# GalDude33/Fetal-MRI-Segmentation

Measured on NVIDIA B200. Metric: U-Net train voxels/sec, higher is better.
Workload: dtype bf16

## Files before the change

fetal-mri-segmentation_b200/csrc/bandwidth.cu:

```cuda
#include "common.cuh"

#include <algorithm>

namespace {

constexpr int kThreads = 256;

__device__ __forceinline__ uint4 ldg16(const void* p) { return __ldg(reinterpret_cast<const uint4*>(p)); }
__device__ __forceinline__ void stg16(void* p, uint4 v) { *reinterpret_cast<uint4*>(p) = v; }

__device__ __forceinline__ void unpack8(uint4 v, float f[8]) {
  const __nv_bfloat162* h = reinterpret_cast<const __nv_bfloat162*>(&v);
#pragma unroll
  for (int i = 0; i < 4; ++i) {
    float2 t = __bfloat1622float2(h[i]);
    f[2 * i] = t.x;
    f[2 * i + 1] = t.y;
  }
}
__device__ __forceinline__ uint4 pack8(const float f[8]) {
  uint4 v;
  __nv_bfloat162* h = reinterpret_cast<__nv_bfloat162*>(&v);
#pragma unroll
  for (int i = 0; i < 4; ++i) h[i] = __floats2bfloat162_rn(f[2 * i], f[2 * i + 1]);
  return v;
}

__global__ void cast_f32_bf16_kernel(const float* __restrict__ in, bf16* __restrict__ out, int64_t n) {
  int64_t i = ((int64_t)blockIdx.x * blockDim.x + threadIdx.x) * 8;
  if (i + 8 <= n) {
    float4 a = __ldg(reinterpret_cast<const float4*>(in + i));
    float4 b = __ldg(reinterpret_cast<const float4*>(in + i + 4));
    float f[8] = {a.x, a.y, a.z, a.w, b.x, b.y, b.z, b.w};
    stg16(out + i, pack8(f));
  } else {
    for (; i < n; ++i) out[i] = __float2bfloat16(in[i]);
  }
}
__global__ void cast_bf16_f32_kernel(const bf16* __restrict__ in, float* __restrict__ out, int64_t n) {
  int64_t i = ((int64_t)blockIdx.x * blockDim.x + threadIdx.x) * 8;
  if (i + 8 <= n) {
    float f[8];
    unpack8(ldg16(in + i), f);
    *reinterpret_cast<float4*>(out + i) = make_float4(f[0], f[1], f[2], f[3]);
    *reinterpret_cast<float4*>(out + i + 4) = make_float4(f[4], f[5], f[6], f[7]);
  } else {
    for (; i < n; ++i) out[i] = __bfloat162float(in[i]);
  }
}

__global__ void pad_cast_kernel(const float* __restrict__ in, bf16* __restrict__ out, int64_t vox, int Cin, int Cpad) {
  const int64_t total = vox * Cpad;
  for (int64_t g = (int64_t)blockIdx.x * blockDim.x + threadIdx.x; g < total; g += (int64_t)gridDim.x * blockDim.x) {
    const int c = (int)(g % Cpad);
    const int64_t v = g / Cpad;
    out[g] = __float2bfloat16(c < Cin ? __ldg(in + v * Cin + c) : 0.f);
  }
}

template <int pz>
__global__ void maxpool3d_fwd_kernel(const bf16* __restrict__ x, bf16* __restrict__ y, int N, int X,
                                     int Y, int Z, int C) {
  FM_PDL_SYNC();
  const int c8n = C >> 3;
  const int Xo = X >> 1, Yo = Y >> 1, Zo = Z / pz;
  const int64_t total = (int64_t)N * Xo * Yo * Zo * c8n;
  int64_t g = (int64_t)blockIdx.x * blockDim.x + threadIdx.x;
  if (g >= total) return;
  const int c8 = (int)(g % c8n);
  int64_t v = g / c8n;
  const int zo = (int)(v % Zo);
  v /= Zo;
  const int yo = (int)(v % Yo);
  v /= Yo;
  const int xo = (int)(v % Xo);
  const int n = (int)(v / Xo);
  __nv_bfloat162 m[4];
  bool first = true;
#pragma unroll
  for (int dx = 0; dx < 2; ++dx)
#pragma unroll
    for (int dy = 0; dy < 2; ++dy)
#pragma unroll
      for (int dz = 0; dz < 2; ++dz) {
        if (dz >= pz) continue;
        const int64_t vi = (((int64_t)n * X + 2 * xo + dx) * Y + 2 * yo + dy) * Z + pz * zo + dz;
        uint4 t = ldg16(x + vi * C + c8 * 8);
        const __nv_bfloat162* h = reinterpret_cast<const __nv_bfloat162*>(&t);
        if (first) {
#pragma unroll
          for (int i = 0; i < 4; ++i) m[i] = h[i];
          first = false;
        } else {
#pragma unroll
          for (int i = 0; i < 4; ++i) m[i] = __hmax2(m[i], h[i]);
        }
      }
  uint4 o;
  __nv_bfloat162* oh = reinterpret_cast<__nv_bfloat162*>(&o);
#pragma unroll
  for (int i = 0; i < 4; ++i) oh[i] = m[i];
  const int64_t vo = (((int64_t)n * Xo + xo) * Yo + yo) * Zo + zo;
  stg16(y + vo * C + c8 * 8, o);
}

template <int pz>
__global__ void __launch_bounds__(kThreads, 4) maxpool3d_bwd_kernel(const bf16* __restrict__ x,
                                                                    const bf16* __restrict__ dy,
                                     const bf16* __restrict__ dskip, bf16* __restrict__ dx, int N,
                                     int X, int Y, int Z, int C, int relu_mask) {
  FM_PDL_SYNC();
  const int c8n = C >> 3;
  const int Xo = X >> 1, Yo = Y >> 1, Zo = Z / pz;
  const int64_t total = (int64_t)N * Xo * Yo * Zo * c8n * 2;
  int64_t g = (int64_t)blockIdx.x * blockDim.x + threadIdx.x;
  const bool live = g < total;
  if (!live) g = total - 2 + (threadIdx.x & 1);
  const int half = (int)(g & 1);
  int64_t v = g >> 1;
  const int c8 = (int)(v % c8n);
  v /= c8n;
  const int zo = (int)(v % Zo);
  v /= Zo;
  const int yo = (int)(v % Yo);
  v /= Yo;
  const int xo = (int)(v % Xo);
  const int n = (int)(v / Xo);
  const int64_t base = ((((int64_t)n * X + 2 * xo + half) * Y + 2 * yo) * Z + pz * zo) * C + c8 * 8;
  const int sy = Z * C;
#define FM_CHILD_OFS(j) (base + (((j) >> 1) * sy + ((j) & 1) * C))
  uint4 xr[4], sk[4];
#pragma unroll
  for (int j = 0; j < 4; ++j) {
    if ((j & 1) < pz) {
      xr[j] = ldg16(x + FM_CHILD_OFS(j));
      sk[j] = dskip != nullptr ? ldg16(dskip + FM_CHILD_OFS(j)) : make_uint4(0u, 0u, 0u, 0u);
    }
  }
  const int64_t vo = (((int64_t)n * Xo + xo) * Yo + yo) * Zo + zo;
  float g8[8];
  unpack8(ldg16(dy + vo * C + c8 * 8), g8);
  float best[8];
  int arg[8];
  unpack8(xr[0], best);
#pragma unroll
  for (int c = 0; c < 8; ++c) arg[c] = 0;
#pragma unroll
  for (int j = 1; j < 4; ++j) {
    if ((j & 1) >= pz) continue;
    float t[8];
    unpack8(xr[j], t);
#pragma unroll
    for (int c = 0; c < 8; ++c)
      if (t[c] > best[c]) {
        best[c] = t[c];
        arg[c] = j;
      }
  }
#pragma unroll
  for (int c = 0; c < 8; ++c) {
    const float other = __shfl_xor_sync(0xffffffffu, best[c], 1);
    const bool mine = half == 0 ? best[c] >= other : best[c] > other;
    if (!mine) arg[c] = -1;
  }
  if (!live) return;
#pragma unroll
  for (int j = 0; j < 4; ++j) {
    if ((j & 1) >= pz) continue;
    float o[8], t[8];
    unpack8(sk[j], o);
    unpack8(xr[j], t);
#pragma unroll
    for (int c = 0; c < 8; ++c) {
      if (arg[c] == j) o[c] += g8[c];
      if (relu_mask && !(t[c] > 0.f)) o[c] = 0.f;
    }
    stg16(dx + FM_CHILD_OFS(j), pack8(o));
  }
#undef FM_CHILD_OFS
}

template <int pz>
__global__ void upsample3d_fwd_kernel(const bf16* __restrict__ x, bf16* __restrict__ y, int N, int X,
                                      int Y, int Z, int C) {
  FM_PDL_SYNC();
  const int c8n = C >> 3;
  const int64_t total = (int64_t)N * X * Y * Z * c8n;
  int64_t g = (int64_t)blockIdx.x * blockDim.x + threadIdx.x;
  if (g >= total) return;
  const int c8 = (int)(g % c8n);
  int64_t v = g / c8n;
  const int z = (int)(v % Z);
  int64_t r = v / Z;
  const int yy = (int)(r % Y);
  r /= Y;
  const int xx = (int)(r % X);
  const int n = (int)(r / X);
  const uint4 t = ldg16(x + v * C + c8 * 8);
  const int X2 = 2 * X, Y2 = 2 * Y, Z2 = pz * Z;
#pragma unroll
  for (int k = 0; k < 8; ++k) {
    const int ddx = k >> 2, ddy = (k >> 1) & 1, ddz = k & 1;
    if (ddz >= pz) continue;
    const int64_t vo = (((int64_t)n * X2 + 2 * xx + ddx) * Y2 + 2 * yy + ddy) * Z2 + pz * z + ddz;
    stg16(y + vo * C + c8 * 8, t);
  }
}

template <int pz>
__global__ void upsample3d_bwd_kernel(const bf16* __restrict__ dy, const bf16* __restrict__ act,
                                      bf16* __restrict__ dx, int N, int X, int Y, int Z, int C,
                                      int dyC, int dy_cofs) {
  FM_PDL_SYNC();
  const int c8n = C >> 3;
  const int64_t total = (int64_t)N * X * Y * Z * c8n;
  int64_t g = (int64_t)blockIdx.x * blockDim.x + threadIdx.x;
  if (g >= total) return;
  const int c8 = (int)(g % c8n);
  int64_t v = g / c8n;
  const int z = (int)(v % Z);
  int64_t r = v / Z;
  const int yy = (int)(r % Y);
  r /= Y;
  const int xx = (int)(r % X);
  const int n = (int)(r / X);
  const int X2 = 2 * X, Y2 = 2 * Y, Z2 = pz * Z;
  float acc[8];
#pragma unroll
  for (int c = 0; c < 8; ++c) acc[c] = 0.f;
#pragma unroll
  for (int k = 0; k < 8; ++k) {
    const int ddx = k >> 2, ddy = (k >> 1) & 1, ddz = k & 1;
    if (ddz >= pz) continue;
    const int64_t vo = (((int64_t)n * X2 + 2 * xx + ddx) * Y2 + 2 * yy + ddy) * Z2 + pz * z + ddz;
    float f[8];
    unpack8(ldg16(dy + vo * dyC + dy_cofs + c8 * 8), f);
#pragma unroll
    for (int c = 0; c < 8; ++c) acc[c] += f[c];
  }
  if (act != nullptr) {
    float a[8];
    unpack8(ldg16(act + v * C + c8 * 8), a);
#pragma unroll
    for (int c = 0; c < 8; ++c)
      if (!(a[c] > 0.f)) acc[c] = 0.f;
  }
  stg16(dx + v * C + c8 * 8, pack8(acc));
}


__device__ __forceinline__ bool fold_channel_groups(float a[8], float b[8], float* sh, int c8n) {
  const int lane = threadIdx.x & 31, warp = threadIdx.x >> 5;
  if (c8n < 32) {
    for (int o = c8n; o < 32; o <<= 1)
#pragma unroll
      for (int i = 0; i < 8; ++i) {
        a[i] += __shfl_xor_sync(0xffffffffu, a[i], o);
        b[i] += __shfl_xor_sync(0xffffffffu, b[i], o);
      }
    if (lane < c8n)
#pragma unroll
      for (int i = 0; i < 8; ++i) {
        sh[(warp * c8n + lane) * 16 + i] = a[i];
// ... 738 lines not shown
  const int64_t pvox = (int64_t)gm.pred[0] * gm.pred[1] * gm.pred[2];
  const uint32_t z4n = (uint32_t)gm.out[2] >> 2;
  const uint32_t plane4 = (uint32_t)gm.out[1] * z4n;
  for (int x = x_lo + blockIdx.y; x < x_hi; x += gridDim.y) {
    const int2 cx = __ldg(reinterpret_cast<const int2*>(cover + (0 * cover_pitch + x) * 2));
    for (uint32_t q = blockIdx.x * blockDim.x + threadIdx.x; q < plane4; q += gridDim.x * blockDim.x) {
      const int z = (int)(q % z4n) * 4;
      const int y = (int)(q / z4n);
      const int2 cy = __ldg(reinterpret_cast<const int2*>(cover + (1 * cover_pitch + y) * 2));
      int2 cz[4];
#pragma unroll
      for (int e = 0; e < 4; ++e) cz[e] = __ldg(reinterpret_cast<const int2*>(cover + (2 * cover_pitch + z + e) * 2));
      double acc[4] = {0.0, 0.0, 0.0, 0.0};
      for (int ix = cx.x; ix < cx.y; ++ix) {
        const int px = x - __ldg(starts + 0 * starts_pitch + ix);
        for (int iy = cy.x; iy < cy.y; ++iy) {
          const int py = y - __ldg(starts + 1 * starts_pitch + iy);
          const int64_t prow = ((int64_t)px * gm.pred[1] + py) * gm.pred[2];
          const int64_t pxy = ((int64_t)ix * gm.np[1] + iy) * gm.np[2];
#pragma unroll
          for (int e = 0; e < 4; ++e)
            for (int iz = cz[e].x; iz < cz[e].y; ++iz) {
              const int64_t patch = pxy + iz;
              if (patch < shard_lo || patch >= shard_hi) continue;
              const int pz = z + e - __ldg(starts + 2 * starts_pitch + iz);
              acc[e] += (double)__ldg(preds + (patch - pred_base) * pvox + prow + pz);
            }
        }
      }
      const int64_t v = ((int64_t)x * gm.out[1] + y) * gm.out[2] + z;
      const int nxy = (cx.y - cx.x) * (cy.y - cy.x);
      double res[4];
      short cn[4];
#pragma unroll
      for (int e = 0; e < 4; ++e) {
        const int cnt = nxy * (cz[e].y - cz[e].x);
        cn[e] = (short)cnt;
        if (!divide) {
          res[e] = out[v + e] + acc[e];
        } else if ((cnt & (cnt - 1)) == 0) {
          res[e] = acc[e] * __longlong_as_double((long long)(1023 - (31 - __clz(cnt))) << 52);
        } else {
          res[e] = acc[e] / (double)cnt;
        }
      }
      reinterpret_cast<double2*>(out + v)[0] = make_double2(res[0], res[1]);
      reinterpret_cast<double2*>(out + v)[1] = make_double2(res[2], res[3]);
      if (count != nullptr) *reinterpret_cast<short4*>(count + v) = make_short4(cn[0], cn[1], cn[2], cn[3]);
    }
  }
}

__global__ void divide_by_count_kernel(double* __restrict__ out, const int16_t* __restrict__ count,
                                       int64_t nvox, int channels) {
  const int64_t total = nvox * channels;
  for (int64_t g = (int64_t)blockIdx.x * blockDim.x + threadIdx.x; g < total;
       g += (int64_t)gridDim.x * blockDim.x)
    out[g] = out[g] / (double)count[g / channels];
}

inline int grid_for(int64_t work_items, int cap = 1 << 30) {
  int64_t b = ceil_div64(work_items, kThreads);
  if (b > cap) b = cap;
  if (b < 1) b = 1;
  return (int)b;
}

}

int k_cast_f32_to_bf16(fm_ctx* ctx, const float* in, bf16* out, int64_t n) {
  cast_f32_bf16_kernel<<<grid_for(ceil_div64(n, 8)), kThreads, 0, ctx->stream>>>(in, out, n);
  FM_LAUNCH_OK(ctx);
  return FM_OK;
}
int k_cast_bf16_to_f32(fm_ctx* ctx, const bf16* in, float* out, int64_t n) {
  cast_bf16_f32_kernel<<<grid_for(ceil_div64(n, 8)), kThreads, 0, ctx->stream>>>(in, out, n);
  FM_LAUNCH_OK(ctx);
  return FM_OK;
}

int k_maxpool3d_fwd(fm_ctx* ctx, const bf16* x, bf16* y, Dims5 in, int pz) {
  FM_CHECK(in.C % 8 == 0 && in.X % 2 == 0 && in.Y % 2 == 0 && in.Z % pz == 0 && (pz == 1 || pz == 2), FM_EINVAL,
           "maxpool3d: need C%%8==0 and even extents (got C=%d %dx%dx%d)", in.C, in.X, in.Y, in.Z);
  const int64_t total = in.elems() / (32 * pz);
  ProfScope prof(ctx, "maxpool3d_fwd", 0.0, (double)in.elems() * 2.0 * 1.125);
  if (pz == 2)
    FM_CUDA(launch_pdl(maxpool3d_fwd_kernel<2>, dim3(grid_for(total)), dim3(kThreads), 0, ctx->stream, x, y, in.N, in.X, in.Y, in.Z, in.C));
  else
    FM_CUDA(launch_pdl(maxpool3d_fwd_kernel<1>, dim3(grid_for(total)), dim3(kThreads), 0, ctx->stream, x, y, in.N, in.X, in.Y, in.Z, in.C));
  FM_LAUNCH_OK(ctx);
  return FM_OK;
}
int k_maxpool3d_bwd(fm_ctx* ctx, const bf16* x, const bf16* dy, const bf16* dskip, bf16* dx, Dims5 in,
                    int relu_mask, int pz) {
  FM_CHECK(in.C % 8 == 0 && in.X % 2 == 0 && in.Y % 2 == 0 && in.Z % pz == 0 && (pz == 1 || pz == 2), FM_EINVAL,
           "maxpool3d_bwd: need C%%8==0 and even extents");
  const int64_t total = in.elems() / (32 * pz) * 2;
  ProfScope prof(ctx, "maxpool3d_bwd", 0.0, (double)in.elems() * 2.0 * (dskip ? 3.125 : 2.125));
  if (pz == 2)
    FM_CUDA(launch_pdl(maxpool3d_bwd_kernel<2>, dim3(grid_for(total)), dim3(kThreads), 0, ctx->stream, x, dy, dskip, dx, in.N, in.X, in.Y, in.Z,
                                                                          in.C, relu_mask));
  else
    FM_CUDA(launch_pdl(maxpool3d_bwd_kernel<1>, dim3(grid_for(total)), dim3(kThreads), 0, ctx->stream, x, dy, dskip, dx, in.N, in.X, in.Y, in.Z,
                                                                          in.C, relu_mask));
  FM_LAUNCH_OK(ctx);
  return FM_OK;
}
int k_upsample3d_fwd(fm_ctx* ctx, const bf16* x, bf16* y, Dims5 in, int pz) {
  FM_CHECK(in.C % 8 == 0, FM_EINVAL, "upsample3d: need C%%8==0");
  ProfScope prof(ctx, "upsample3d_fwd", 0.0, (double)in.elems() * 2.0 * 9.0);
  if (pz == 2)
    FM_CUDA(launch_pdl(upsample3d_fwd_kernel<2>, dim3(grid_for(in.elems() / 8)), dim3(kThreads), 0, ctx->stream, x, y, in.N, in.X, in.Y, in.Z, in.C));
  else
    FM_CUDA(launch_pdl(upsample3d_fwd_kernel<1>, dim3(grid_for(in.elems() / 8)), dim3(kThreads), 0, ctx->stream, x, y, in.N, in.X, in.Y, in.Z, in.C));
  FM_LAUNCH_OK(ctx);
  return FM_OK;
}
int k_upsample3d_bwd(fm_ctx* ctx, const bf16* dy, const bf16* act, bf16* dx, Dims5 coarse, int dy_C,
                     int dy_cofs, int pz) {
  FM_CHECK(coarse.C % 8 == 0 && dy_C % 8 == 0 && dy_cofs % 8 == 0, FM_EINVAL,
           "upsample3d_bwd: channel counts must be multiples of 8");
  ProfScope prof(ctx, "upsample3d_bwd", 0.0, (double)coarse.elems() * 2.0 * (act ? 10.0 : 9.0));
  if (pz == 2)
    FM_CUDA(launch_pdl(upsample3d_bwd_kernel<2>, dim3(grid_for(coarse.elems() / 8)), dim3(kThreads), 0, ctx->stream, 
        dy, act, dx, coarse.N, coarse.X, coarse.Y, coarse.Z, coarse.C, dy_C, dy_cofs));
  else
    FM_CUDA(launch_pdl(upsample3d_bwd_kernel<1>, dim3(grid_for(coarse.elems() / 8)), dim3(kThreads), 0, ctx->stream, 
        dy, act, dx, coarse.N, coarse.X, coarse.Y, coarse.Z, coarse.C, dy_C, dy_cofs));
  FM_LAUNCH_OK(ctx);
  return FM_OK;
}

int k_dice_sums(fm_ctx* ctx, const float* p, const float* t, int64_t n, double* sums, int accumulate, XentSpec xs) {
  ProfScope prof(ctx, "dice_sums", 0.0, (double)n * (xs.mask ? 12.0 : 8.0));
  FM_CUDA(launch_pdl(dice_partial_kernel, dim3(kRedBlocks), dim3(kThreads), 0, ctx->stream, p, t, n, ctx->red_scratch, xs));
  FM_LAUNCH_OK(ctx);
  FM_CUDA(launch_pdl(dice_final_kernel, dim3(1), dim3(256), 0, ctx->stream, ctx->red_scratch, kRedBlocks, (double)n, sums,
                                              accumulate));
  FM_LAUNCH_OK(ctx);
  return FM_OK;
}
int k_dice_finalize(fm_ctx* ctx, int nblocks, double n_elems, double* sums) {
  FM_CUDA(launch_pdl(dice_final_kernel, dim3(1), dim3(256), 0, ctx->stream, ctx->red_scratch, nblocks, n_elems, sums, 0));
  FM_LAUNCH_OK(ctx);
  return FM_OK;
}
int k_dice_bwd(fm_ctx* ctx, const float* p, const float* t, const double* sums, int64_t n, float* dz,
               int through_sigmoid, XentSpec xs) {
  FM_CHECK(xs.weight == 0.f || through_sigmoid, FM_EINVAL, "dice_bwd: the cross-entropy term is formed through the sigmoid");
  ProfScope prof(ctx, "dice_bwd", 0.0, (double)n * (xs.mask ? 16.0 : 12.0));
  FM_CUDA(launch_pdl(dice_bwd_kernel, dim3(grid_for(ceil_div64(n, 4))), dim3(kThreads), 0, ctx->stream, p, t, sums, n, dz,
                                                                           through_sigmoid, xs));
  FM_LAUNCH_OK(ctx);
  return FM_OK;
}
int k_adam(fm_ctx* ctx, float* p, const float* g, float* m, float* v, int64_t n, int iterations,
           float lr) {
  const double b1 = 0.9, b2 = 0.999;
  const double t = (double)iterations + 1.0;
  const float lr_t = (float)((double)lr * sqrt(1.0 - pow(b2, t)) / (1.0 - pow(b1, t)));
  ProfScope prof(ctx, "adam", 0.0, (double)n * 28.0);
  FM_CUDA(launch_pdl(adam_kernel, dim3(grid_for(ceil_div64(n, 4))), dim3(kThreads), 0, ctx->stream, p, g, m, v, n, lr_t, 0.9f,
                                                                       0.999f, 1e-7f));
  FM_LAUNCH_OK(ctx);
  return FM_OK;
}
int k_zero(fm_ctx* ctx, void* p, size_t bytes) {
  FM_CUDA(cudaMemsetAsync(p, 0, bytes, ctx->stream));
  return FM_OK;
}

int k_pad_cast(fm_ctx* ctx, const float* in, bf16* out, int64_t vox, int Cin, int Cpad) {
  ProfScope prof(ctx, "pad_cast", 0.0, (double)vox * (Cin * 4.0 + Cpad * 2.0));
  pad_cast_kernel<<<grid_for(vox * Cpad, 148 * 32), kThreads, 0, ctx->stream>>>(in, out, vox, Cin, Cpad);
  FM_LAUNCH_OK(ctx);
  return FM_OK;
}

int k_gather_patches(fm_ctx* ctx, const float* vol, const int32_t vol_dims[3],
                     const int32_t halo_pad[6], const int32_t fit_pad[6], float pad0, float pad1,
// ... 474 lines not shown
```

fetal-mri-segmentation_b200/csrc/conv_first_tc.cu:

```cuda
#include <algorithm>

#include "tc_ptx.cuh"

using namespace tcp;

namespace {

constexpr int kFY = 16, kFZ = 8;
constexpr int kBuildWarps = 4;
constexpr int kThreadsF = 32 * (kBuildWarps + 1 + 4);
constexpr uint32_t kATile = 128u * 128u;
constexpr int kABufs = 3;
constexpr int kDyRingF = 4;

struct alignas(64) FirstParams {
  CUtensorMap tmDY;
  const float* x;
  const bf16* w;
  const float* bias;
  bf16* y;
  float* dw;
  int N, X, Y, Z, Cout, relu;
  int ty, tz, tiles;
};

__device__ __forceinline__ void fence_async_smem() { asm volatile("fence.proxy.async.shared::cta;" ::: "memory"); }

constexpr int kHZ = 12;
constexpr uint32_t kHaloBytes = 3u * 18u * kHZ * 2u;
constexpr int kHaloPerThread = 5;

__device__ __forceinline__ void halo_load(const FirstParams& p, int n, int x, int y0, int z0, int tid, float v[kHaloPerThread]) {
#pragma unroll
  for (int k = 0; k < kHaloPerThread; ++k) {
    const int e = tid + k * 128;
    const int kx = e / 180, rem = e % 180;
    const int yy = rem / 10, zz = rem % 10;
    const int xi = x + kx - 1, yi = y0 + yy - 1, zi = z0 + zz - 1;
    const bool ok = e < 540 && xi >= 0 && xi < p.X && yi >= 0 && yi < p.Y && zi >= 0 && zi < p.Z;
    v[k] = ok ? __ldg(p.x + (((int64_t)n * p.X + xi) * p.Y + yi) * p.Z + zi) : 0.f;
  }
}
__device__ __forceinline__ void halo_store(uint32_t halo, int tid, const float v[kHaloPerThread]) {
#pragma unroll
  for (int k = 0; k < kHaloPerThread; ++k) {
    const int e = tid + k * 128;
    if (e < 540) {
      const int kx = e / 180, rem = e % 180;
      const int yy = rem / 10, zz = rem % 10;
      const bf16 h = __float2bfloat16(v[k]);
      asm volatile("st.shared.u16 [%0], %1;" ::"r"(halo + (uint32_t)(((kx * 18 + yy) * kHZ + zz) * 2)),
                   "h"(*reinterpret_cast<const unsigned short*>(&h))
                   : "memory");
    }
  }
}
__device__ __forceinline__ void build_row(uint32_t halo, uint32_t tile, int row, int ry, int rz) {
  uint32_t h[28];
#pragma unroll
  for (int kx = 0; kx < 3; ++kx)
#pragma unroll
    for (int ky = 0; ky < 3; ++ky) {
      const uint32_t a = halo + (uint32_t)(((kx * 18 + ry + ky) * kHZ + rz) * 2);
#pragma unroll
      for (int kz = 0; kz < 3; ++kz) {
        unsigned short u;
        asm volatile("ld.shared.u16 %0, [%1];" : "=h"(u) : "r"(a + 2u * (uint32_t)kz));
        h[(kx * 3 + ky) * 3 + kz] = u;
      }
    }
  h[27] = 0u;
  const uint32_t rbase = tile + (uint32_t)row * 128u;
  const uint32_t sw = (uint32_t)(row & 7);
#pragma unroll
  for (int c = 0; c < 4; ++c) {
    uint32_t w4[4];
#pragma unroll
    for (int j = 0; j < 4; ++j) {
      const int t = 8 * c + 2 * j;
      w4[j] = t + 1 < 28 ? (h[t] | (h[t + 1] << 16)) : (t < 28 ? h[t] : 0u);
    }
    asm volatile("st.shared.v4.u32 [%0], {%1, %2, %3, %4};" ::"r"(rbase + (((uint32_t)c ^ sw) << 4)), "r"(w4[0]),
                 "r"(w4[1]), "r"(w4[2]), "r"(w4[3])
                 : "memory");
  }
}

__device__ __forceinline__ void decode_tile(const FirstParams& p, int tile, int& n, int& x, int& y0, int& z0) {
  const int iz = tile % p.tz;
  int t = tile / p.tz;
  const int iy = t % p.ty;
  t /= p.ty;
  x = t % p.X;
  n = t / p.X;
  y0 = iy * kFY;
  z0 = iz * kFZ;
}

template <int MODE>
__global__ void __launch_bounds__(kThreadsF, 1) conv3d_first_tc_kernel(const __grid_constant__ FirstParams p) {
  extern __shared__ uint8_t smem_raw[];
  const uint32_t smem0 = (smem_u32(smem_raw) + 1023u) & ~1023u;
  const int warp = threadIdx.x >> 5, lane = threadIdx.x & 31;
  const uint32_t a_base = smem0;
  const uint32_t w_base = a_base + (uint32_t)(kABufs + 1) * kATile;
  const uint32_t dy_tile = 128u * (uint32_t)p.Cout * 2u;
  const uint32_t halo_base = w_base + (MODE == 0 ? 32u * 128u : (uint32_t)kDyRingF * dy_tile);
  const uint32_t bar0 = (halo_base + 2u * kHaloBytes + 15u) & ~15u;
  auto afull = [&](int b) { return bar0 + 8u * (uint32_t)b; };
  auto aempty = [&](int b) { return bar0 + 8u * (uint32_t)(kABufs + b); };
  auto tfull = [&](int a) { return bar0 + 8u * (uint32_t)(2 * kABufs + a); };
  auto tempty = [&](int a) { return bar0 + 8u * (uint32_t)(2 * kABufs + 2 + a); };
  auto dyfull = [&](int s) { return bar0 + 8u * (uint32_t)(2 * kABufs + 4 + s); };
  auto dyempty = [&](int s) { return bar0 + 8u * (uint32_t)(2 * kABufs + 4 + kDyRingF + s); };
  const uint32_t tmem_slot = bar0 + 8u * (uint32_t)(2 * kABufs + 4 + 2 * kDyRingF);
  const uint32_t tmem_cols = MODE == 0 ? (p.Cout == 16 ? 32u : 64u) : 32u;

  for (uint32_t i = threadIdx.x; i < (uint32_t)(kABufs + 1) * kATile / 16u; i += blockDim.x)
    asm volatile("st.shared.v4.u32 [%0], {%1, %1, %1, %1};" ::"r"(a_base + i * 16u), "r"(0u) : "memory");
  if (MODE == 0) {
    for (uint32_t i = threadIdx.x; i < 32u * 128u / 16u; i += blockDim.x)
      asm volatile("st.shared.v4.u32 [%0], {%1, %1, %1, %1};" ::"r"(w_base + i * 16u), "r"(0u) : "memory");
  }
  __syncthreads();
  if (MODE == 0) {
    for (int i = threadIdx.x; i < p.Cout * 27; i += blockDim.x) {
      const int co = i / 27, t = i % 27;
      const uint32_t addr = w_base + (uint32_t)co * 128u + ((((uint32_t)t >> 3) ^ (uint32_t)(co & 7)) << 4) + ((uint32_t)t & 7u) * 2u;
      const bf16 wv = p.w[i];
      asm volatile("st.shared.u16 [%0], %1;" ::"r"(addr), "h"(*reinterpret_cast<const unsigned short*>(&wv)) : "memory");
    }
  }
  if (warp == kBuildWarps) {
    if (lane == 0) {
      for (int b = 0; b < kABufs; ++b) {
        mbar_init(afull(b), kBuildWarps * 32);
        mbar_init(aempty(b), 1);
      }
      for (int a = 0; a < 2; ++a) {
        mbar_init(tfull(a), 1);
        mbar_init(tempty(a), 128);
      }
      for (int s = 0; s < kDyRingF; ++s) {
        mbar_init(dyfull(s), 1);
        mbar_init(dyempty(s), 1);
      }
      fence_barrier_init();
      if (MODE == 1) prefetch_tmap(&p.tmDY);
    }
    __syncwarp();
    tmem_alloc(tmem_slot, tmem_cols);
  }
  fence_async_smem();
  tc_fence_before();
  __syncthreads();
  tc_fence_after();
  uint32_t tmem_base;
  asm volatile("ld.shared.u32 %0, [%1];" : "=r"(tmem_base) : "r"(tmem_slot));
  tmem_base = __shfl_sync(0xffffffffu, tmem_base, 0);
  const int warp_u = __shfl_sync(0xffffffffu, warp, 0);

  if (warp_u < kBuildWarps) {
    pdl_wait();
    if (warp_u == 0) pdl_launch_dependents();
    const int row = threadIdx.x;
    const int ry = row / kFZ, rz = row % kFZ;
    float hv[kHaloPerThread];
    int n, x, y0, z0;
    if ((int)blockIdx.x < p.tiles) {
      decode_tile(p, blockIdx.x, n, x, y0, z0);
      halo_load(p, n, x, y0, z0, row, hv);
    }
    uint32_t it = 0;
    for (int tile = blockIdx.x; tile < p.tiles; tile += gridDim.x, ++it) {
      const uint32_t b = it % (uint32_t)kABufs, ph = (it / (uint32_t)kABufs) & 1u;
      const uint32_t halo = halo_base + (it & 1u) * kHaloBytes;
      halo_store(halo, row, hv);
      const int next = tile + gridDim.x;
      if (next < p.tiles) {
        decode_tile(p, next, n, x, y0, z0);
        halo_load(p, n, x, y0, z0, row, hv);
      }
      asm volatile("bar.sync 1, 128;" ::: "memory");
      mbar_wait(aempty(b), ph ^ 1u);
      build_row(halo, a_base + b * kATile, row, ry, rz);
      fence_async_smem();
      mbar_arrive(afull(b));
    }
  } else if (warp_u == kBuildWarps) {
    const uint32_t a_hi = desc_hi(1024u, layout_code(128));
    uint32_t it = 0;
    if (MODE == 0) {
      const uint32_t idesc = make_idesc(128, p.Cout, 0, 0);
      const uint32_t b_lo = desc_lo(w_base, 16u);
      for (int tile = blockIdx.x; tile < p.tiles; tile += gridDim.x, ++it) {
        const uint32_t b = it % (uint32_t)kABufs, ph = (it / (uint32_t)kABufs) & 1u;
        const uint32_t acc = it & 1u, acc_ph = (it >> 1) & 1u;
        mbar_wait(tempty(acc), acc_ph ^ 1u);
        mbar_wait(afull(b), ph);
        tc_fence_after();
        const uint32_t a_lo = desc_lo(a_base + b * kATile, 16u);
        const uint32_t d = tmem_base + acc * (uint32_t)p.Cout;
        umma_bf16_lh_elect(d, a_lo, a_hi, b_lo, a_hi, idesc, 0u);
        umma_bf16_lh_elect(d, a_lo + 2u, a_hi, b_lo + 2u, a_hi, idesc, 1u);
        umma_commit_elect(aempty(b));
        umma_commit_elect(tfull(acc));
      }
    } else {
      pdl_wait();
      const uint32_t idesc = make_idesc(128, p.Cout, 1, 1);
      const uint32_t b_row = (uint32_t)p.Cout * 2u, b_sbo = 8u * b_row;
      const uint32_t b_hi = desc_hi(b_sbo, layout_code((int)b_row));
      const uint32_t b_step = (2u * b_sbo) >> 4;
      int ahead = blockIdx.x;
      uint32_t issued = 0;
      auto issue_dy = [&]() {
        if (ahead >= p.tiles) return;
        const uint32_t s = issued % (uint32_t)kDyRingF, sph = (issued / (uint32_t)kDyRingF) & 1u;
        int n, x, y0, z0;
        decode_tile(p, ahead, n, x, y0, z0);
        mbar_wait(dyempty(s), sph ^ 1u);
        mbar_expect_tx_elect(dyfull(s), dy_tile);
        tma_load_5d_elect(w_base + s * dy_tile, &p.tmDY, dyfull(s), 0, z0, y0, x, n);
        ++issued;
        ahead += gridDim.x;
      };
      for (int i = 0; i < kDyRingF - 1; ++i) issue_dy();
      for (int tile = blockIdx.x; tile < p.tiles; tile += gridDim.x, ++it) {
        issue_dy();
        const uint32_t b = it % (uint32_t)kABufs, ph = (it / (uint32_t)kABufs) & 1u;
        const uint32_t s = it % (uint32_t)kDyRingF, sph = (it / (uint32_t)kDyRingF) & 1u;
        mbar_wait(afull(b), ph);
        mbar_wait(dyfull(s), sph);
        tc_fence_after();
        uint32_t a_lo = desc_lo(a_base + b * kATile, kATile);
        uint32_t b_lo = desc_lo(w_base + s * dy_tile, dy_tile);
#pragma unroll
        for (int ks = 0; ks < 8; ++ks) {
          umma_bf16_lh_elect(tmem_base, a_lo, a_hi, b_lo, b_hi, idesc, (it > 0 || ks > 0) ? 1u : 0u);
          a_lo += 128u;
          b_lo += b_step;
        }
        umma_commit_elect(aempty(b));
        umma_commit_elect(dyempty(s));
      }
      umma_commit_elect(tfull(0));
    }
  } else {
    const int q = warp & 3;
    const int row = q * 32 + lane;
    const uint32_t lane_base = tmem_base + ((uint32_t)(q * 32) << 16);
    if (MODE == 0) {
      const int ry = row / kFZ, rz = row % kFZ;
      uint32_t it = 0;
      for (int tile = blockIdx.x; tile < p.tiles; tile += gridDim.x, ++it) {
        const uint32_t acc = it & 1u, acc_ph = (it >> 1) & 1u;
        int n, x, y0, z0;
        decode_tile(p, tile, n, x, y0, z0);
        const int64_t v = (((int64_t)n * p.X + x) * p.Y + y0 + ry) * p.Z + z0 + rz;
        mbar_wait(tfull(acc), acc_ph);
        tc_fence_after();
        for (int c16 = 0; c16 < p.Cout / 16; ++c16) {
          uint32_t r[16];
          tmem_ld16(lane_base + acc * (uint32_t)p.Cout + (uint32_t)c16 * 16u, r);
          tmem_ld_wait();
          uint4 o[2];
          __nv_bfloat162* oh = reinterpret_cast<__nv_bfloat162*>(o);
#pragma unroll
          for (int j = 0; j < 8; ++j) {
            float a = __uint_as_float(r[2 * j]) + __ldg(p.bias + c16 * 16 + 2 * j);
            float b = __uint_as_float(r[2 * j + 1]) + __ldg(p.bias + c16 * 16 + 2 * j + 1);
            if (p.relu) {
              a = fmaxf(a, 0.f);
              b = fmaxf(b, 0.f);
            }
            oh[j] = __floats2bfloat162_rn(a, b);
          }
          uint4* op = reinterpret_cast<uint4*>(p.y + v * p.Cout + c16 * 16);
          op[0] = o[0];
          op[1] = o[1];
        }
        tc_fence_before();
        mbar_arrive(tempty(acc));
      }
    } else {
      mbar_wait(tfull(0), 0);
      tc_fence_after();
      if ((int)blockIdx.x < p.tiles) {
        for (int c16 = 0; c16 < p.Cout / 16; ++c16) {
          uint32_t r[16];
          tmem_ld16(lane_base + (uint32_t)c16 * 16u, r);
          tmem_ld_wait();
          if (row < 27) {
#pragma unroll
            for (int j = 0; j < 16; ++j) atomicAdd(p.dw + (c16 * 16 + j) * 27 + row, __uint_as_float(r[j]));
          }
        }
      }
    }
  }

  tc_fence_before();
  __syncthreads();
  if (warp == kBuildWarps) {
    tc_fence_after();
    tmem_dealloc(tmem_base, tmem_cols);
  }
}

size_t first_smem(int mode, int Cout) {
  return (size_t)(kABufs + 1) * kATile + (mode == 0 ? 32u * 128u : (size_t)kDyRingF * 128u * Cout * 2u) + 2 * kHaloBytes +
         1024 + 256 + 16;
}

int fill(FirstParams& p, int N, int X, int Y, int Z, int Cout) {
  memset(&p, 0, sizeof(p));
  p.N = N;
  p.X = X;
  p.Y = Y;
  p.Z = Z;
  p.Cout = Cout;
  p.ty = Y / kFY;
  p.tz = Z / kFZ;
  p.tiles = N * X * p.ty * p.tz;
  return FM_OK;
}

}

int conv_first_tc_supported(int X, int Y, int Z, int Cout) {
  return X > 0 && Y % kFY == 0 && Z % kFZ == 0 && (Cout == 16 || Cout == 32);
}

int k_conv3d_first_tc(fm_ctx* ctx, const float* x, const bf16* w_packed, const float* bias, bf16* y, int N, int X, int Y,
                      int Z, int Cout, int relu) {
  FM_CHECK(conv_first_tc_supported(X, Y, Z, Cout) && bias != nullptr, FM_EINVAL, "conv3d first tc: unsupported %dx%dx%d Cout=%d",
           X, Y, Z, Cout);
  FirstParams p;
  FM_TRY(fill(p, N, X, Y, Z, Cout));
  p.x = x;
  p.w = w_packed;
  p.bias = bias;
  p.y = y;
  p.relu = relu;
  const size_t smem = first_smem(0, Cout);
  static bool attr_set = false;
  if (!attr_set) {
    FM_CUDA(cudaFuncSetAttribute(conv3d_first_tc_kernel<0>, cudaFuncAttributeMaxDynamicSharedMemorySize, (int)first_smem(0, 32)));
    attr_set = true;
  }
  const double nvox = (double)N * X * Y * Z;
  const int grid = std::min(p.tiles, 3 * ctx->num_sms);
  ProfScope prof(ctx, "conv3d_first", 2.0 * 27 * Cout * nvox, nvox * (4.0 + 2.0 * Cout));
  FM_CUDA(launch_pdl(conv3d_first_tc_kernel<0>, dim3(grid), dim3(kThreadsF), smem, ctx->stream, p));
  FM_LAUNCH_OK(ctx);
  return FM_OK;
}

int k_conv3d_first_tc_wgrad(fm_ctx* ctx, const float* x, const bf16* dy, float* dw, int N, int X, int Y, int Z, int Cout) {
  FM_CHECK(conv_first_tc_supported(X, Y, Z, Cout), FM_EINVAL, "conv3d first tc wgrad: unsupported %dx%dx%d Cout=%d", X, Y, Z,
           Cout);
  FirstParams p;
  FM_TRY(fill(p, N, X, Y, Z, Cout));
  p.x = x;
  p.dw = dw;
  EncodeTiledFn enc = encode_tiled();
  FM_CHECK(enc != nullptr, FM_ECUDA, "cuTensorMapEncodeTiled entry point not available");
  cuuint64_t dims[5] = {(cuuint64_t)Cout, (cuuint64_t)Z, (cuuint64_t)Y, (cuuint64_t)X, (cuuint64_t)N};
  cuuint64_t strides[4] = {(cuuint64_t)Cout * 2, (cuuint64_t)Z * Cout * 2, (cuuint64_t)Y * Z * Cout * 2,
                           (cuuint64_t)X * Y * Z * Cout * 2};
  cuuint32_t box[5] = {(cuuint32_t)Cout, (cuuint32_t)kFZ, (cuuint32_t)kFY, 1, 1};
  cuuint32_t estr[5] = {1, 1, 1, 1, 1};
  CUresult r = enc(&p.tmDY, CU_TENSOR_MAP_DATA_TYPE_BFLOAT16, 5, (void*)dy, dims, strides, box, estr,
                   CU_TENSOR_MAP_INTERLEAVE_NONE, swizzle_for_row_bytes(Cout * 2),
                   CU_TENSOR_MAP_L2_PROMOTION_L2_256B, CU_TENSOR_MAP_FLOAT_OOB_FILL_NONE);
  FM_CHECK(r == CUDA_SUCCESS, FM_ECUDA, "cuTensorMapEncodeTiled(first wgrad) failed: %d", (int)r);
  const size_t smem = first_smem(1, Cout);
  static bool attr_set = false;
  if (!attr_set) {
    FM_CUDA(cudaFuncSetAttribute(conv3d_first_tc_kernel<1>, cudaFuncAttributeMaxDynamicSharedMemorySize, (int)first_smem(1, 32)));
    attr_set = true;
  }
  const double nvox = (double)N * X * Y * Z;
  const int grid = std::min(p.tiles, 2 * ctx->num_sms);
  ProfScope prof(ctx, "conv3d_first_wgrad", 2.0 * 27 * Cout * nvox, nvox * (4.0 + 2.0 * Cout));
  FM_CUDA(launch_pdl(conv3d_first_tc_kernel<1>, dim3(grid), dim3(kThreadsF), smem, ctx->stream, p));
  FM_LAUNCH_OK(ctx);
  return FM_OK;
}
```

Baseline: 657.4 million.

## Split maxpool windows across z-pair lanes and deepen first-conv halo and dY prefetch

Maxpool forward and backward now use one lane per z-slice of each 2x2x2 window, with a shared index helper. Partial maxima and argmax results are combined across the lane pair by warp shuffles, and the backward pass packs argmax into a bitfield with tie-breaking. The backward launch bound drops from 4 to 3 blocks per SM. Separately, the first-layer tensor-core conv now prefetches halos four tiles ahead instead of one, and sizes its dY TMA ring by a fixed byte budget, which gives more stages when Cout is 16. All of this aims to raise memory-level parallelism in bandwidth-bound kernels, at the cost of more registers and extra shuffles.

```diff
diff --git a/fetal-mri-segmentation_b200/csrc/bandwidth.cu b/fetal-mri-segmentation_b200/csrc/bandwidth.cu
--- a/fetal-mri-segmentation_b200/csrc/bandwidth.cu
+++ b/fetal-mri-segmentation_b200/csrc/bandwidth.cu
@@ -58,66 +58,24 @@
   }
 }
 
+struct PoolLane {
+  int64_t base;
+  int64_t vo;
+  int ddz;
+  bool live;
+};
+
 template <int pz>
-__global__ void maxpool3d_fwd_kernel(const bf16* __restrict__ x, bf16* __restrict__ y, int N, int X,
-                                     int Y, int Z, int C) {
-  FM_PDL_SYNC();
+__device__ __forceinline__ PoolLane pool_lane(int N, int X, int Y, int Z, int C) {
   const int c8n = C >> 3;
   const int Xo = X >> 1, Yo = Y >> 1, Zo = Z / pz;
-  const int64_t total = (int64_t)N * Xo * Yo * Zo * c8n;
+  const int64_t total = (int64_t)N * Xo * Yo * Zo * c8n * pz;
   int64_t g = (int64_t)blockIdx.x * blockDim.x + threadIdx.x;
-  if (g >= total) return;
-  const int c8 = (int)(g % c8n);
-  int64_t v = g / c8n;
-  const int zo = (int)(v % Zo);
-  v /= Zo;
-  const int yo = (int)(v % Yo);
-  v /= Yo;
-  const int xo = (int)(v % Xo);
-  const int n = (int)(v / Xo);
-  __nv_bfloat162 m[4];
-  bool first = true;
-#pragma unroll
-  for (int dx = 0; dx < 2; ++dx)
-#pragma unroll
-    for (int dy = 0; dy < 2; ++dy)
-#pragma unroll
-      for (int dz = 0; dz < 2; ++dz) {
-        if (dz >= pz) continue;
-        const int64_t vi = (((int64_t)n * X + 2 * xo + dx) * Y + 2 * yo + dy) * Z + pz * zo + dz;
-        uint4 t = ldg16(x + vi * C + c8 * 8);
-        const __nv_bfloat162* h = reinterpret_cast<const __nv_bfloat162*>(&t);
-        if (first) {
-#pragma unroll
-          for (int i = 0; i < 4; ++i) m[i] = h[i];
-          first = false;
-        } else {
-#pragma unroll
-          for (int i = 0; i < 4; ++i) m[i] = __hmax2(m[i], h[i]);
-        }
-      }
-  uint4 o;
-  __nv_bfloat162* oh = reinterpret_cast<__nv_bfloat162*>(&o);
-#pragma unroll
-  for (int i = 0; i < 4; ++i) oh[i] = m[i];
-  const int64_t vo = (((int64_t)n * Xo + xo) * Yo + yo) * Zo + zo;
-  stg16(y + vo * C + c8 * 8, o);
-}
-
-template <int pz>
-__global__ void __launch_bounds__(kThreads, 4) maxpool3d_bwd_kernel(const bf16* __restrict__ x,
-                                                                    const bf16* __restrict__ dy,
-                                     const bf16* __restrict__ dskip, bf16* __restrict__ dx, int N,
-                                     int X, int Y, int Z, int C, int relu_mask) {
-  FM_PDL_SYNC();
-  const int c8n = C >> 3;
-  const int Xo = X >> 1, Yo = Y >> 1, Zo = Z / pz;
-  const int64_t total = (int64_t)N * Xo * Yo * Zo * c8n * 2;
-  int64_t g = (int64_t)blockIdx.x * blockDim.x + threadIdx.x;
-  const bool live = g < total;
-  if (!live) g = total - 2 + (threadIdx.x & 1);
-  const int half = (int)(g & 1);
-  int64_t v = g >> 1;
+  PoolLane l;
+  l.live = g < total;
+  if (!l.live) g = total - pz + (threadIdx.x & (pz - 1));
+  l.ddz = pz == 2 ? (int)(g & 1) : 0;
+  int64_t v = pz == 2 ? g >> 1 : g;
   const int c8 = (int)(v % c8n);
   v /= c8n;
   const int zo = (int)(v % Zo);
@@ -126,59 +84,96 @@
   v /= Yo;
   const int xo = (int)(v % Xo);
   const int n = (int)(v / Xo);
-  const int64_t base = ((((int64_t)n * X + 2 * xo + half) * Y + 2 * yo) * Z + pz * zo) * C + c8 * 8;
-  const int sy = Z * C;
-#define FM_CHILD_OFS(j) (base + (((j) >> 1) * sy + ((j) & 1) * C))
+  l.base = ((((int64_t)n * X + 2 * xo) * Y + 2 * yo) * Z + pz * zo + l.ddz) * C + c8 * 8;
+  l.vo = ((((int64_t)n * Xo + xo) * Yo + yo) * Zo + zo) * C + c8 * 8;
+  return l;
+}
+#define FM_CHILD_OFS(l, j) ((l).base + ((j) >> 1) * (int64_t)Y * Z * C + ((j) & 1) * (int64_t)Z * C)
+
+template <int pz>
+__global__ void maxpool3d_fwd_kernel(const bf16* __restrict__ x, bf16* __restrict__ y, int N, int X,
+                                     int Y, int Z, int C) {
+  FM_PDL_SYNC();
+  const PoolLane l = pool_lane<pz>(N, X, Y, Z, C);
+  uint4 xr[4];
+#pragma unroll
+  for (int j = 0; j < 4; ++j) xr[j] = ldg16(x + FM_CHILD_OFS(l, j));
+  __nv_bfloat162 m[4];
+  const __nv_bfloat162* h0 = reinterpret_cast<const __nv_bfloat162*>(&xr[0]);
+#pragma unroll
+  for (int i = 0; i < 4; ++i) m[i] = h0[i];
+#pragma unroll
+  for (int j = 1; j < 4; ++j) {
+    const __nv_bfloat162* h = reinterpret_cast<const __nv_bfloat162*>(&xr[j]);
+#pragma unroll
+    for (int i = 0; i < 4; ++i) m[i] = __hmax2(m[i], h[i]);
+  }
+  uint32_t* mu = reinterpret_cast<uint32_t*>(m);
+  if (pz == 2) {
+#pragma unroll
+    for (int i = 0; i < 4; ++i) {
+      const uint32_t o = __shfl_xor_sync(0xffffffffu, mu[i], 1);
+      m[i] = __hmax2(m[i], *reinterpret_cast<const __nv_bfloat162*>(&o));
+    }
+  }
+  if (!l.live || l.ddz != 0) return;
+  stg16(y + l.vo, make_uint4(mu[0], mu[1], mu[2], mu[3]));
+}
+
+template <int pz>
+__global__ void __launch_bounds__(kThreads, 3) maxpool3d_bwd_kernel(const bf16* __restrict__ x,
+                                                                    const bf16* __restrict__ dy,
+                                     const bf16* __restrict__ dskip, bf16* __restrict__ dx, int N,
+                                     int X, int Y, int Z, int C, int relu_mask) {
+  FM_PDL_SYNC();
+  const PoolLane l = pool_lane<pz>(N, X, Y, Z, C);
   uint4 xr[4], sk[4];
 #pragma unroll
   for (int j = 0; j < 4; ++j) {
-    if ((j & 1) < pz) {
-      xr[j] = ldg16(x + FM_CHILD_OFS(j));
-      sk[j] = dskip != nullptr ? ldg16(dskip + FM_CHILD_OFS(j)) : make_uint4(0u, 0u, 0u, 0u);
-    }
-  }
-  const int64_t vo = (((int64_t)n * Xo + xo) * Yo + yo) * Zo + zo;
+    xr[j] = ldg16(x + FM_CHILD_OFS(l, j));
+    sk[j] = dskip != nullptr ? ldg16(dskip + FM_CHILD_OFS(l, j)) : make_uint4(0u, 0u, 0u, 0u);
+  }
   float g8[8];
-  unpack8(ldg16(dy + vo * C + c8 * 8), g8);
+  unpack8(ldg16(dy + l.vo), g8);
   float best[8];
-  int arg[8];
+  uint32_t arg = 0, win = 0xffu;
   unpack8(xr[0], best);
 #pragma unroll
-  for (int c = 0; c < 8; ++c) arg[c] = 0;
-#pragma unroll
   for (int j = 1; j < 4; ++j) {
-    if ((j & 1) >= pz) continue;
     float t[8];
     unpack8(xr[j], t);
 #pragma unroll
     for (int c = 0; c < 8; ++c)
       if (t[c] > best[c]) {
         best[c] = t[c];
-        arg[c] = j;
+        arg = (arg & ~(3u << (2 * c))) | ((uint32_t)j << (2 * c));
       }
   }
-#pragma unroll
-  for (int c = 0; c < 8; ++c) {
-    const float other = __shfl_xor_sync(0xffffffffu, best[c], 1);
-    const bool mine = half == 0 ? best[c] >= other : best[c] > other;
-    if (!mine) arg[c] = -1;
-  }
-  if (!live) return;
+  if (pz == 2) {
+    const uint32_t oarg = __shfl_xor_sync(0xffffffffu, arg, 1);
+#pragma unroll
+    for (int c = 0; c < 8; ++c) {
+      const float other = __shfl_xor_sync(0xffffffffu, best[c], 1);
+      const uint32_t a = (arg >> (2 * c)) & 3u, oa = (oarg >> (2 * c)) & 3u;
+      const bool first = l.ddz == 0 ? a <= oa : a < oa;
+      if (!(best[c] > other || (best[c] == other && first))) win &= ~(1u << c);
+    }
+  }
+  if (!l.live) return;
 #pragma unroll
   for (int j = 0; j < 4; ++j) {
-    if ((j & 1) >= pz) continue;
     float o[8], t[8];
     unpack8(sk[j], o);
     unpack8(xr[j], t);
 #pragma unroll
     for (int c = 0; c < 8; ++c) {
-      if (arg[c] == j) o[c] += g8[c];
+      if (((win >> c) & 1u) && ((arg >> (2 * c)) & 3u) == (uint32_t)j) o[c] += g8[c];
       if (relu_mask && !(t[c] > 0.f)) o[c] = 0.f;
     }
-    stg16(dx + FM_CHILD_OFS(j), pack8(o));
-  }
+    stg16(dx + FM_CHILD_OFS(l, j), pack8(o));
+  }
+}
 #undef FM_CHILD_OFS
-}
 
 template <int pz>
 __global__ void upsample3d_fwd_kernel(const bf16* __restrict__ x, bf16* __restrict__ y, int N, int X,
@@ -1083,7 +1078,7 @@
 int k_maxpool3d_fwd(fm_ctx* ctx, const bf16* x, bf16* y, Dims5 in, int pz) {
   FM_CHECK(in.C % 8 == 0 && in.X % 2 == 0 && in.Y % 2 == 0 && in.Z % pz == 0 && (pz == 1 || pz == 2), FM_EINVAL,
            "maxpool3d: need C%%8==0 and even extents (got C=%d %dx%dx%d)", in.C, in.X, in.Y, in.Z);
-  const int64_t total = in.elems() / (32 * pz);
+  const int64_t total = in.elems() / 32;
   ProfScope prof(ctx, "maxpool3d_fwd", 0.0, (double)in.elems() * 2.0 * 1.125);
   if (pz == 2)
     FM_CUDA(launch_pdl(maxpool3d_fwd_kernel<2>, dim3(grid_for(total)), dim3(kThreads), 0, ctx->stream, x, y, in.N, in.X, in.Y, in.Z, in.C));
@@ -1096,7 +1091,7 @@
                     int relu_mask, int pz) {
   FM_CHECK(in.C % 8 == 0 && in.X % 2 == 0 && in.Y % 2 == 0 && in.Z % pz == 0 && (pz == 1 || pz == 2), FM_EINVAL,
            "maxpool3d_bwd: need C%%8==0 and even extents");
-  const int64_t total = in.elems() / (32 * pz) * 2;
+  const int64_t total = in.elems() / 32;
   ProfScope prof(ctx, "maxpool3d_bwd", 0.0, (double)in.elems() * 2.0 * (dskip ? 3.125 : 2.125));
   if (pz == 2)
     FM_CUDA(launch_pdl(maxpool3d_bwd_kernel<2>, dim3(grid_for(total)), dim3(kThreads), 0, ctx->stream, x, dy, dskip, dx, in.N, in.X, in.Y, in.Z,
diff --git a/fetal-mri-segmentation_b200/csrc/conv_first_tc.cu b/fetal-mri-segmentation_b200/csrc/conv_first_tc.cu
--- a/fetal-mri-segmentation_b200/csrc/conv_first_tc.cu
+++ b/fetal-mri-segmentation_b200/csrc/conv_first_tc.cu
@@ -11,7 +11,8 @@
 constexpr int kThreadsF = 32 * (kBuildWarps + 1 + 4);
 constexpr uint32_t kATile = 128u * 128u;
 constexpr int kABufs = 3;
-constexpr int kDyRingF = 4;
+constexpr uint32_t kDyRingBytes = 32768;
+constexpr int kDyRingMax = 8;
 
 struct alignas(64) FirstParams {
   CUtensorMap tmDY;
@@ -29,6 +30,7 @@
 constexpr int kHZ = 12;
 constexpr uint32_t kHaloBytes = 3u * 18u * kHZ * 2u;
 constexpr int kHaloPerThread = 5;
+constexpr int kHaloDepth = 4;
 
 __device__ __forceinline__ void halo_load(const FirstParams& p, int n, int x, int y0, int z0, int tid, float v[kHaloPerThread]) {
 #pragma unroll
@@ -105,15 +107,16 @@
   const uint32_t a_base = smem0;
   const uint32_t w_base = a_base + (uint32_t)(kABufs + 1) * kATile;
   const uint32_t dy_tile = 128u * (uint32_t)p.Cout * 2u;
-  const uint32_t halo_base = w_base + (MODE == 0 ? 32u * 128u : (uint32_t)kDyRingF * dy_tile);
+  const int dy_ring = (int)(kDyRingBytes / dy_tile);
+  const uint32_t halo_base = w_base + (MODE == 0 ? 32u * 128u : kDyRingBytes);
   const uint32_t bar0 = (halo_base + 2u * kHaloBytes + 15u) & ~15u;
   auto afull = [&](int b) { return bar0 + 8u * (uint32_t)b; };
   auto aempty = [&](int b) { return bar0 + 8u * (uint32_t)(kABufs + b); };
   auto tfull = [&](int a) { return bar0 + 8u * (uint32_t)(2 * kABufs + a); };
   auto tempty = [&](int a) { return bar0 + 8u * (uint32_t)(2 * kABufs + 2 + a); };
   auto dyfull = [&](int s) { return bar0 + 8u * (uint32_t)(2 * kABufs + 4 + s); };
-  auto dyempty = [&](int s) { return bar0 + 8u * (uint32_t)(2 * kABufs + 4 + kDyRingF + s); };
-  const uint32_t tmem_slot = bar0 + 8u * (uint32_t)(2 * kABufs + 4 + 2 * kDyRingF);
+  auto dyempty = [&](int s) { return bar0 + 8u * (uint32_t)(2 * kABufs + 4 + kDyRingMax + s); };
+  const uint32_t tmem_slot = bar0 + 8u * (uint32_t)(2 * kABufs + 4 + 2 * kDyRingMax);
   const uint32_t tmem_cols = MODE == 0 ? (p.Cout == 16 ? 32u : 64u) : 32u;
 
   for (uint32_t i = threadIdx.x; i < (uint32_t)(kABufs + 1) * kATile / 16u; i += blockDim.x)
@@ -141,7 +144,7 @@
         mbar_init(tfull(a), 1);
         mbar_init(tempty(a), 128);
       }
-      for (int s = 0; s < kDyRingF; ++s) {
+      for (int s = 0; s < dy_ring; ++s) {
         mbar_init(dyfull(s), 1);
         mbar_init(dyempty(s), 1);
       }
@@ -165,27 +168,36 @@
     if (warp_u == 0) pdl_launch_dependents();
     const int row = threadIdx.x;
     const int ry = row / kFZ, rz = row % kFZ;
-    float hv[kHaloPerThread];
+    float hv[kHaloDepth][kHaloPerThread];
     int n, x, y0, z0;
-    if ((int)blockIdx.x < p.tiles) {
-      decode_tile(p, blockIdx.x, n, x, y0, z0);
-      halo_load(p, n, x, y0, z0, row, hv);
+#pragma unroll
+    for (int d = 0; d < kHaloDepth; ++d) {
+      const int t = (int)blockIdx.x + d * (int)gridDim.x;
+      if (t < p.tiles) {
+        decode_tile(p, t, n, x, y0, z0);
+        halo_load(p, n, x, y0, z0, row, hv[d]);
+      }
     }
     uint32_t it = 0;
-    for (int tile = blockIdx.x; tile < p.tiles; tile += gridDim.x, ++it) {
-      const uint32_t b = it % (uint32_t)kABufs, ph = (it / (uint32_t)kABufs) & 1u;
-      const uint32_t halo = halo_base + (it & 1u) * kHaloBytes;
-      halo_store(halo, row, hv);
-      const int next = tile + gridDim.x;
-      if (next < p.tiles) {
-        decode_tile(p, next, n, x, y0, z0);
-        halo_load(p, n, x, y0, z0, row, hv);
-      }
-      asm volatile("bar.sync 1, 128;" ::: "memory");
-      mbar_wait(aempty(b), ph ^ 1u);
-      build_row(halo, a_base + b * kATile, row, ry, rz);
-      fence_async_smem();
-      mbar_arrive(afull(b));
+    for (int tile0 = blockIdx.x; tile0 < p.tiles; tile0 += kHaloDepth * gridDim.x) {
+#pragma unroll
+      for (int d = 0; d < kHaloDepth; ++d, ++it) {
+        const int tile = tile0 + d * (int)gridDim.x;
+        if (tile >= p.tiles) break;
+        const uint32_t b = it % (uint32_t)kABufs, ph = (it / (uint32_t)kABufs) & 1u;
+        const uint32_t halo = halo_base + (it & 1u) * kHaloBytes;
+        halo_store(halo, row, hv[d]);
+        const int next = tile + kHaloDepth * (int)gridDim.x;
+        if (next < p.tiles) {
+          decode_tile(p, next, n, x, y0, z0);
+          halo_load(p, n, x, y0, z0, row, hv[d]);
+        }
+        asm volatile("bar.sync 1, 128;" ::: "memory");
+        mbar_wait(aempty(b), ph ^ 1u);
+        build_row(halo, a_base + b * kATile, row, ry, rz);
+        fence_async_smem();
+        mbar_arrive(afull(b));
+      }
     }
   } else if (warp_u == kBuildWarps) {
     const uint32_t a_hi = desc_hi(1024u, layout_code(128));
@@ -216,7 +228,7 @@
       uint32_t issued = 0;
       auto issue_dy = [&]() {
         if (ahead >= p.tiles) return;
-        const uint32_t s = issued % (uint32_t)kDyRingF, sph = (issued / (uint32_t)kDyRingF) & 1u;
+        const uint32_t s = issued % (uint32_t)dy_ring, sph = (issued / (uint32_t)dy_ring) & 1u;
         int n, x, y0, z0;
         decode_tile(p, ahead, n, x, y0, z0);
         mbar_wait(dyempty(s), sph ^ 1u);
@@ -225,11 +237,11 @@
         ++issued;
         ahead += gridDim.x;
       };
-      for (int i = 0; i < kDyRingF - 1; ++i) issue_dy();
+      for (int i = 0; i < dy_ring - 1; ++i) issue_dy();
       for (int tile = blockIdx.x; tile < p.tiles; tile += gridDim.x, ++it) {
         issue_dy();
         const uint32_t b = it % (uint32_t)kABufs, ph = (it / (uint32_t)kABufs) & 1u;
-        const uint32_t s = it % (uint32_t)kDyRingF, sph = (it / (uint32_t)kDyRingF) & 1u;
+        const uint32_t s = it % (uint32_t)dy_ring, sph = (it / (uint32_t)dy_ring) & 1u;
         mbar_wait(afull(b), ph);
         mbar_wait(dyfull(s), sph);
         tc_fence_after();
@@ -308,9 +320,8 @@
   }
 }
 
-size_t first_smem(int mode, int Cout) {
-  return (size_t)(kABufs + 1) * kATile + (mode == 0 ? 32u * 128u : (size_t)kDyRingF * 128u * Cout * 2u) + 2 * kHaloBytes +
-         1024 + 256 + 16;
+size_t first_smem(int mode) {
+  return (size_t)(kABufs + 1) * kATile + (mode == 0 ? 32u * 128u : (size_t)kDyRingBytes) + 2 * kHaloBytes + 1024 + 256 + 16;
 }
 
 int fill(FirstParams& p, int N, int X, int Y, int Z, int Cout) {
@@ -343,10 +354,10 @@
   p.bias = bias;
   p.y = y;
   p.relu = relu;
-  const size_t smem = first_smem(0, Cout);
+  const size_t smem = first_smem(0);
   static bool attr_set = false;
   if (!attr_set) {
-    FM_CUDA(cudaFuncSetAttribute(conv3d_first_tc_kernel<0>, cudaFuncAttributeMaxDynamicSharedMemorySize, (int)first_smem(0, 32)));
+    FM_CUDA(cudaFuncSetAttribute(conv3d_first_tc_kernel<0>, cudaFuncAttributeMaxDynamicSharedMemorySize, (int)first_smem(0)));
     attr_set = true;
   }
   const double nvox = (double)N * X * Y * Z;
@@ -375,10 +386,10 @@
                    CU_TENSOR_MAP_INTERLEAVE_NONE, swizzle_for_row_bytes(Cout * 2),
                    CU_TENSOR_MAP_L2_PROMOTION_L2_256B, CU_TENSOR_MAP_FLOAT_OOB_FILL_NONE);
   FM_CHECK(r == CUDA_SUCCESS, FM_ECUDA, "cuTensorMapEncodeTiled(first wgrad) failed: %d", (int)r);
-  const size_t smem = first_smem(1, Cout);
+  const size_t smem = first_smem(1);
   static bool attr_set = false;
   if (!attr_set) {
-    FM_CUDA(cudaFuncSetAttribute(conv3d_first_tc_kernel<1>, cudaFuncAttributeMaxDynamicSharedMemorySize, (int)first_smem(1, 32)));
+    FM_CUDA(cudaFuncSetAttribute(conv3d_first_tc_kernel<1>, cudaFuncAttributeMaxDynamicSharedMemorySize, (int)first_smem(1)));
     attr_set = true;
   }
   const double nvox = (double)N * X * Y * Z;
```

Result: faster. 664.7 million, median of 6 (+1.1%).
